# GonzaBerger/bmSparse-SPGEMM-SPMV

Hardware: AMD Instinct MI355X
Metric: bmSparse SpMV fp32 effective GB/s (CSR-convention bytes / time); SpGEMM GFLOP/s under `spgemm` (higher is better)
Workload: dtype f32; 1 GPU; bmSparse SpMV fp32, rmat(scale=20, edge_factor=2)+I, stand-in for webbase-1M; rows=1048576, nnz=3127380, blocks=2073692, x=ones, variant=default (value-stream sweep over the cached plan), hbm_resident_copies_rotated=9

## Files before the change

### bmsparse-spgemm-spmv_amd/csrc/builder.hip

```cpp
#include "matrix.h"
#include "prims.hip.h"
#include <algorithm>
#include <cctype>
#include <memory>
#include <thread>
#include <string>
#include <cstdlib>
#include <cerrno>
#include <cstring>
#include <fcntl.h>
#include <sys/mman.h>
#include <sys/stat.h>
#include <unistd.h>

namespace bmsp {

namespace {
struct MappedFile {
    const char *p = nullptr;
    size_t n = 0;
    int fd = -1;
    ~MappedFile()
    {
        if (p && n) munmap((void *)p, n);
// ... 379 lines not shown
    BMSP_HIP(hipDeviceSynchronize());
    pool_free(m->dense_tiles); m->dense_tiles = nullptr;
    pool_free(m->lane_tiles); m->lane_tiles = nullptr;
    pool_free(m->csr_rowptr); pool_free(m->csr_ent);
    m->csr_rowptr = nullptr; m->csr_ent = nullptr;
    m->values_finite = -1;
    if (!structure_changed) return;
    pool_free(m->rowptr); m->rowptr = nullptr; m->rowptr_rows = 0; m->max_row_blocks = -1;
    m->struct_hash = 0; m->sp_a_hash = 0; m->sp_b_hash = 0;
    m->rm_partner_uid = 0; m->rm_partner_blocks = 0; m->rm_partner_mode = 0; m->rm_partner_cw_hash = 0;
    m->uid = next_matrix_uid();
    pool_free(m->sp_tasks); pool_free(m->sp_task_begin); pool_free(m->sp_c_of_wave);
    m->sp_tasks = nullptr; m->sp_task_begin = nullptr; m->sp_c_of_wave = nullptr; m->sp_n_tasks = 0;
    pool_free(m->spmv_chunks); m->spmv_chunks = nullptr; m->spmv_num_chunks = 0; m->spmv_plan_long = 0; m->spmv_full_tiles = 0;
    pool_free(m->spmv_pos); m->spmv_pos = nullptr; m->spmv_tinfo = nullptr; m->spmv_eoff = nullptr; m->spmv_pos_base = 0; m->spmv_pos_count = 0; m->spmv_pos_tried = 0;
    pool_free(m->spmv_cw); m->spmv_cw = nullptr; m->spmv_cw_chunks = 0; m->spmv_cw_split = 0; m->spmv_cw_tried = 0;
    pool_free(m->block_meta); m->block_meta = nullptr;
    pool_free(m->sym_recs); m->sym_recs = nullptr;
    pool_free(m->col_index); pool_free(m->col_index_row); m->col_index = nullptr; m->col_index_row = nullptr; m->col_index_tried = 0;
    pool_free(m->col_mass); m->col_mass = nullptr;
    pool_free(m->tp_map); m->tp_map = nullptr; m->tp_src_uid = 0; m->tp_permute = 0;
    pool_free(m->add_map); m->add_map = nullptr; m->add_a_uid = 0; m->add_b_uid = 0;
    free_matrix(m->shard_view); m->shard_view = nullptr; m->shard_world = 0; m->shard_rank = 0; m->shard_bounds.clear();
}

void drop_value_caches(bmsp_matrix_s *m)
{
    if (m->dense_tiles || m->lane_tiles || m->csr_rowptr || m->csr_ent) invalidate_matrix(m, 0);
    else m->values_finite = -1;
}

// ... 535 lines not shown
```

### bmsparse-spgemm-spmv_amd/csrc/capi.hip

```cpp
#include "matrix.h"
#include "prims.hip.h"
#include <algorithm>
#include <cmath>
#include <cstdio>
#include <cstdlib>
#include <cstring>
#include <memory>
#include <numeric>
#include <omp.h>
#include <vector>

namespace bmsp {
const std::string &last_error();
void partition_rows(bmsp_matrix_s *A, bmsp_matrix_s *B, int parts, int64_t *bounds, hipStream_t st, uint64_t *total_out = nullptr);
void spgemm_paneled(bmsp_matrix_s *A, bmsp_matrix_s *B, bmsp_matrix_s **C, int mode, int tc_version, int verbose, hipStream_t st,
                    bmsp_spgemm_stats *stats);
bmsp_matrix_s *row_panel(bmsp_matrix_s *m, int64_t rb, int64_t re, hipStream_t st);
bmsp_matrix_s *concat_panels(int num_rows, int num_cols, int parts, const int64_t *block_nums, const int64_t *nnzs,
                             uint64_t *const *d_keys, uint64_t *const *d_bmps, uint64_t *const *d_offsets, void *const *d_values,
                             bmsp_dtype dtype, hipStream_t st);
}

using namespace bmsp;

// ... 540 lines not shown
}

int bmsp_spmv(bmsp_matrix_t A, const void *d_v, void *d_u, int variant, void *stream)
{
    BMSP_API_BEGIN
    need(A, "A");
    spmv(A, d_v, d_u, variant, as_stream(stream));
    BMSP_API_END
}

int bmsp_spmv_launch_info(bmsp_matrix_t A, int variant, char *kernel_name, size_t kernel_name_cap, int64_t *compulsory_bytes, int64_t *format_bytes)
{
    BMSP_API_BEGIN
    need(A, "A");
    spmv_launch_info(A, variant, nullptr, kernel_name, kernel_name_cap, compulsory_bytes, format_bytes);
    BMSP_API_END
}

int bmsp_comm_unique_id(void *id_bytes)
{
    BMSP_API_BEGIN
    need(id_bytes, "id_bytes");
    comm_unique_id(id_bytes);
    BMSP_API_END
}

int bmsp_comm_init(const void *id_bytes, int world, int rank, bmsp_comm_t *out)
{
    BMSP_API_BEGIN
    need(id_bytes, "id_bytes"); need(out, "out");
// ... 394 lines not shown
```

### bmsparse-spgemm-spmv_amd/csrc/matrix.h

```cpp
#ifndef BMSP_MATRIX_H_
#define BMSP_MATRIX_H_

#include "runtime.h"
#include <memory>
#include <vector>

namespace bmsp { uint64_t next_matrix_uid(); }

struct bmsp_matrix_s {
    uint64_t uid = bmsp::next_matrix_uid();
    int num_rows = 0, num_cols = 0;
    int64_t nnz = 0, block_num = 0;
    bmsp_dtype dtype = BMSP_F32;
    int transposed = 0;
    uint64_t *keys = nullptr;
    uint64_t *bmps = nullptr;
    uint64_t *offsets = nullptr;
    void *values = nullptr;
    int ownership = 1;
    uint32_t *rowptr = nullptr;
    int64_t rowptr_rows = 0;
    int64_t max_row_blocks = -1;
    uint32_t *spmv_chunks = nullptr;
    int64_t spmv_num_chunks = 0;
    int64_t spmv_plan_long = 0;
    int64_t spmv_full_tiles = 0;
    size_t spmv_plan_off_cnt = 0, spmv_plan_off_carry = 0;
    uint16_t *spmv_pos = nullptr;
    uint32_t *spmv_tinfo = nullptr;
    uint16_t *spmv_eoff = nullptr;
    int64_t spmv_pos_base = 0, spmv_pos_count = 0;
    int spmv_pos_tried = 0;
    uint32_t *spmv_cw = nullptr;
    int64_t spmv_cw_chunks = 0, spmv_cw_split = 0;
    size_t spmv_cw_off_rec = 0, spmv_cw_off_cnt = 0, spmv_cw_off_carry = 0;
    int spmv_cw_colbits = 0, spmv_cw_tried = 0;
    uint32_t *block_meta = nullptr;
    uint32_t *sym_recs = nullptr;
    uint32_t *col_mass = nullptr;
    uint32_t *col_index = nullptr, *col_index_row = nullptr;
    uint32_t col_index_gran = 0;
    int col_index_tried = 0;
    void *dense_tiles = nullptr;
    uint32_t *csr_rowptr = nullptr, *csr_ent = nullptr;
    void *lane_tiles = nullptr;
    uint64_t rm_partner_uid = 0;
    int64_t rm_partner_blocks = 0;
    int rm_partner_mode = 0;
    int64_t rm_partner_cw_hash = 0;
    uint64_t *sp_tasks = nullptr;
    uint32_t *sp_task_begin = nullptr, *sp_c_of_wave = nullptr;
// ... 117 lines not shown
void prune_check_args(int rule, double tol, int flags, int out_transposed);
void prune_matrix(bmsp_matrix_s *A, int rule, double tol, int flags, int out_transposed, hipStream_t st, bmsp_matrix_s **out,
                  bmsp_prune_stats *stats);
void row_absmax(bmsp_matrix_s *A, void *d_rowmax, hipStream_t st);
void scale_check_args(const void *d_left, const void *d_right, int flags, int out_transposed);
void from_diagonal_check_args(int num_rows, int num_cols, const void *d_diag, bmsp_dtype dtype, int transposed);
void matrix_diagonal(bmsp_matrix_s *A, void *d_diag, hipStream_t st);
bmsp_matrix_s *matrix_from_diagonal(int num_rows, int num_cols, const void *d_diag, bmsp_dtype dtype, int transposed, hipStream_t st);
bmsp_matrix_s *scale_matrix(bmsp_matrix_s *A, const void *d_left, const void *d_right, int flags, int out_transposed, hipStream_t st);
void scale_values_into(bmsp_matrix_s *A, const void *d_left, const void *d_right, int flags, bmsp_matrix_s *out, hipStream_t st);
void prepare_spmv(bmsp_matrix_s *m, hipStream_t st);
void prepare_spgemm_operand(bmsp_matrix_s *m, hipStream_t st);

void spmv(bmsp_matrix_s *A, const void *v, void *u, int variant, hipStream_t st, int64_t row_lo = 0, int64_t row_hi = -1);
void spmv_launch_info(bmsp_matrix_s *A, int variant, hipStream_t st, char *kernel, size_t kernel_cap, int64_t *compulsory, int64_t *format_bytes);
void spmm(bmsp_matrix_s *A, const void *X, int64_t ldx, void *Y, int64_t ldy, int k, hipStream_t st);
void spmm_launch_info(bmsp_matrix_s *A, int k, int64_t ldx, int64_t ldy, hipStream_t st, char *kernel, size_t kernel_cap);
void spgemm(bmsp_matrix_s *A, bmsp_matrix_s *B, bmsp_matrix_s **C, int mode, int tc_version, int verbose, hipStream_t st,
            bmsp_spgemm_stats *stats, bool structure_only = false);
void spgemm_numeric(bmsp_matrix_s *A, bmsp_matrix_s *B, bmsp_matrix_s *C, int tc_version, hipStream_t st, bmsp_spgemm_stats *stats);
template <typename T>
struct PingPong;
bool segsort_tasks_by_column(PingPong<uint64_t> &keys, PingPong<uint64_t> &vals, uint64_t n, int jbits, hipStream_t st, uint64_t max_seg_bound = 0,
                             uint64_t seg_count_bound = 0, int *long_mode = nullptr);
void segsort_check_violation();
void segsort_u64(uint64_t *d_keys, void *d_vals, int val_bytes, int64_t n, const int *d_segs, int64_t num_segs,
                 hipStream_t st);

void comm_unique_id(void *id128);
bmsp_comm_s *comm_init(const void *id128, int world, int rank);
// ... 13 lines not shown
```

### bmsparse-spgemm-spmv_amd/csrc/spmv.hip

```cpp
#include "spmv_plan.h"
#include "prims.hip.h"
#include <cstdlib>
#include <cstdio>
#include <algorithm>
#include <vector>
#include <type_traits>

namespace bmsp {
namespace {

constexpr uint32_t kVsGroup = 96;
bool vstream_eligible(const bmsp_matrix_s *A)
{
    return !(A->spmv_full_tiles * 4 >= A->block_num) && !getenv("BMSP_SPMV_OLD") && A->num_block_cols() < (1ll << 28);
}

struct RowClass {
    const uint32_t *rowptr;
    const uint64_t *offsets;
    uint32_t nbr;
    uint32_t group;
    __device__ bool is_long(uint32_t r) const { return rowptr[r + 1] - rowptr[r] > kItemTiles; }
    __device__ bool starts(uint32_t r) const
    {
// ... 1027 lines not shown
        sum = chunk_fold_batch<1>(carry, ca, ca, cb, r, g);
    } else if (n <= 16u) {
        sum = chunk_fold_batch<2>(carry, ca, ca, cb, r, g);
    } else {
        sum = 0.f;
        for (uint32_t kb = ca; kb <= cb; kb += 32u) sum += chunk_fold_batch<4>(carry, ca, kb, cb, r, g);
    }
    sum += dpp_val<0x111>(0.f, sum);
    sum += dpp_val<0x112>(0.f, sum);
    sum += dpp_val<0x114>(0.f, sum);
    const uint32_t row = br * 8u + r;
    if (g == 7u && row < num_rows) y[row] = sum;
    if (lane == 0) __hip_atomic_store(&counters[ca], 0u, __ATOMIC_RELAXED, __HIP_MEMORY_SCOPE_AGENT);
}

__global__ __launch_bounds__(64, 8) void spmv_chunk_kernel(const ChunkRec *__restrict__ recs, const uint32_t *__restrict__ words,
                                                            const float *__restrict__ values, const float *__restrict__ x, float *__restrict__ y,
                                                            float *__restrict__ carry, uint32_t *__restrict__ counters, uint32_t nnz,
                                                            uint32_t num_rows, uint32_t num_cols, uint32_t colbits)
{
    typedef float f4 __attribute__((ext_vector_type(4)));
    typedef uint32_t u4 __attribute__((ext_vector_type(4)));
    __shared__ __attribute__((aligned(16))) float win[kChWin];
    const int lane = lane_id();
    const uint32_t c = blockIdx.x;
    const ChunkRec rc = recs[c];
    const uint32_t first = c * kChV + (uint32_t)(kChPer * lane);
    const rsrc_t rw = make_rsrc(words, nnz * 4u), rv = make_rsrc(values, nnz * 4u), rx = make_rsrc(x, num_cols * 4u);
    uint32_t w[kChPer];
    float a[kChPer], xv[kChPer];
    if (c * kChV + kChV <= nnz) {
#pragma unroll
        for (int q = 0; q < kChPer; q += 4) {
            const u4 wq = __builtin_bit_cast(u4, __builtin_amdgcn_raw_buffer_load_b128(rw, (first + q) * 4u, 0, 0));
            const f4 aq = __builtin_bit_cast(f4, __builtin_amdgcn_raw_buffer_load_b128(rv, (first + q) * 4u, 0, 0));
#pragma unroll
            for (int i = 0; i < 4; i++) { w[q + i] = wq[i]; a[q + i] = aq[i]; }
        }
    } else {
#pragma unroll
        for (int j = 0; j < kChPer; j++) {
            const uint32_t off = first + j < nnz ? (first + j) * 4u : kOob;
            w[j] = __builtin_amdgcn_raw_buffer_load_b32(rw, off, 0, 0);
            a[j] = Buf<float>::ld(rv, off);
        }
    }
    const uint32_t cmask = (1u << colbits) - 1u;
#pragma unroll
    for (int j = 0; j < kChPer; j++) xv[j] = Buf<float>::ld(rx, first + j < nnz ? (w[j] & cmask) * 4u : kOob);

    float pr[kChPer];
    uint32_t rr[kChPer];
#pragma unroll
    for (int j = 0; j < kChPer; j++) {
        rr[j] = first + j < nnz ? w[j] >> colbits : rc.nwin - 8u;
        pr[j] = first + j < nnz ? a[j] * xv[j] : 0.f;
    }
    if (rc.nwin == 8) {
        float s[8] = {0.f, 0.f, 0.f, 0.f, 0.f, 0.f, 0.f, 0.f};
#pragma unroll
        for (int j = 0; j < kChPer; j++) {
#pragma unroll
            for (int k = 0; k < 8; k++) s[k] += rr[j] == (uint32_t)k ? pr[j] : 0.f;
        }
        const float v = chunk_sum8(s, lane);
        if ((lane & 7) == 0) win[((lane >> 5) & 1) * 4 + ((lane >> 4) & 1) * 2 + ((lane >> 3) & 1)] = v;
    } else {
        for (uint32_t e = (uint32_t)lane; e < rc.nwin; e += 64) win[e] = 0.f;
        __builtin_amdgcn_wave_barrier();
        chunk_seg_reduce(win, rr, pr);
    }
    __builtin_amdgcn_wave_barrier();
    uint32_t ticket = 0;
    if (rc.flags) {
        if ((rc.flags & kChHead) && lane < 8) __hip_atomic_store(&carry[((size_t)c * 2) * 8 + lane], win[lane], __ATOMIC_RELAXED, __HIP_MEMORY_SCOPE_AGENT);
        if ((rc.flags & kChTail) && lane < 8)
            __hip_atomic_store(&carry[((size_t)c * 2 + 1) * 8 + lane], win[rc.nwin - 8u + (uint32_t)lane], __ATOMIC_RELAXED, __HIP_MEMORY_SCOPE_AGENT);
        asm volatile("s_waitcnt vmcnt(0)" ::: "memory");
        if (lane == 0 ? (rc.flags & kChHead) != 0u : lane == 1 && (rc.flags & kChTail) != 0u)
            ticket = __hip_atomic_fetch_add(&counters[lane == 0 ? rc.head_ca : c], 1u, __ATOMIC_RELAXED, __HIP_MEMORY_SCOPE_AGENT);
    }
    const int32_t base = (int32_t)(rc.fb * 8u);
    const uint32_t row_end = min(rc.own_e * 8u, num_rows);
    for (uint32_t row = rc.own_b * 8u + (uint32_t)lane; row < row_end; row += 64) {
        const int32_t rel = (int32_t)row - base;
        y[row] = rel >= 0 && rel < (int32_t)rc.nwin ? win[rel] : 0.f;
    }
    if (!rc.flags) return;
    const uint32_t th = (uint32_t)__builtin_amdgcn_readlane((int)ticket, 0), tt = (uint32_t)__builtin_amdgcn_readlane((int)ticket, 1);
    if ((rc.flags & kChHead) && th == rc.head_cb - rc.head_ca) chunk_fold(carry, y, counters, rc.head_ca, rc.head_cb, rc.fb, num_rows, lane);
    if ((rc.flags & kChTail) && tt == rc.tail_cb - c) chunk_fold(carry, y, counters, c, rc.tail_cb, rc.fb + rc.nwin / 8u - 1u, num_rows, lane);
}

__global__ void chunk_bounds_kernel(const uint64_t *__restrict__ keys, const uint64_t *__restrict__ bmps, const uint64_t *__restrict__ offsets,
                                    uint32_t nb, uint32_t nnz, uint32_t *__restrict__ fbr, uint32_t *__restrict__ lbr)
{
    const uint32_t b = blockIdx.x * blockDim.x + threadIdx.x;
    if (b >= nb) return;
    const uint32_t o = (uint32_t)offsets[b], n = (uint32_t)__popcll(bmps[b]);
    if (n == 0) return;
    const uint32_t br = key_row(keys[b]);
// ... 10 lines not shown
    const uint32_t b = blockIdx.x * blockDim.x + threadIdx.x;
    if (b >= nb) return;
    uint64_t bm = bmps[b];
    const uint64_t k = keys[b];
    const uint32_t br = key_row(k), bc = key_col(k);
    uint32_t idx = (uint32_t)offsets[b];
    while (bm) {
        const uint32_t p = (uint32_t)__clzll((long long)bm);
        bm &= ~(0x8000000000000000ull >> p);
        const uint32_t rel = (br - fbr[idx / kChV]) * 8u + (p >> 3);
        words[idx] = (rel << colbits) | (bc * 8u + (p & 7u));
        idx++;
    }
}

void build_chunk_cache(bmsp_matrix_s *A, hipStream_t st)
{
    if (A->spmv_cw || A->spmv_cw_tried) return;
    A->spmv_cw_tried = 1;
    if (A->dtype != BMSP_F32 || A->view_values_end || A->view_block_begin || A->nnz == 0 || A->nnz >= (1ll << 30) || A->block_num == 0) return;
    if ((uintptr_t)A->values & 15u) return;
    const uint32_t nnz = (uint32_t)A->nnz, nb = (uint32_t)A->block_num;
    const uint32_t nch = (nnz + kChV - 1) / kChV;
    const int colbits = A->num_cols <= 1 ? 1 : 32 - __builtin_clz((uint32_t)A->num_cols - 1u);
    if (colbits > 28) return;
    std::vector<uint32_t> fb(nch), lb(nch);
    {
        DevBuf<uint32_t> d(2 * (size_t)nch);
        hipLaunchKernelGGL(chunk_bounds_kernel, dim3((nb + 255) / 256), dim3(256), 0, st, A->keys, A->bmps, A->offsets, nb, nnz, d.p, d.p + nch);
        BMSP_CHECK_LAUNCH();
        BMSP_HIP(hipStreamSynchronize(st));
        copy_d2h_staged(fb.data(), d.p, 4 * (size_t)nch);
        copy_d2h_staged(lb.data(), d.p + nch, 4 * (size_t)nch);
    }
    const uint64_t row_cap = std::min<uint64_t>(kChWin, 1ull << (32 - colbits));
    std::vector<ChunkRec> rec(nch);
    const uint32_t nbr = (uint32_t)A->num_block_rows();
    int64_t split = 0;
    for (uint32_t c = 0; c < nch; c++) {
        ChunkRec &r = rec[c];
// ... 12 lines not shown
        uint32_t e = c + 1;
        while (e + 1 < nch && fb[e + 1] == lb[c]) e++;
        rec[c].tail_cb = e;
        for (uint32_t k = c + 1; k <= e; k++) { rec[k].head_ca = c; rec[k].head_cb = e; }
    }
    const size_t off_rec = (size_t)nch * kChV * 4, off_cnt = off_rec + sizeof(ChunkRec) * (size_t)nch;
    const size_t off_carry = (off_cnt + 4 * (size_t)nch + 63) & ~size_t(63), total = off_carry + 64 * (size_t)nch;
    char *mem = (char *)pool_alloc(total);
    BMSP_HIP(hipMemsetAsync(mem, 0, total, st));
    BMSP_HIP(hipMemcpyAsync(mem + off_rec, rec.data(), sizeof(ChunkRec) * (size_t)nch, hipMemcpyHostToDevice, st));
    {
        DevBuf<uint32_t> d(nch);
        BMSP_HIP(hipMemcpyAsync(d.p, fb.data(), 4 * (size_t)nch, hipMemcpyHostToDevice, st));
        hipLaunchKernelGGL(chunk_words_kernel, dim3((nb + 255) / 256), dim3(256), 0, st, A->keys, A->bmps, A->offsets, nb, d.p, (uint32_t)colbits, (uint32_t *)mem);
        BMSP_CHECK_LAUNCH();
        BMSP_HIP(hipStreamSynchronize(st));
    }
    A->spmv_cw = (uint32_t *)mem;
    A->spmv_cw_chunks = nch;
    A->spmv_cw_split = split;
    A->spmv_cw_off_rec = off_rec; A->spmv_cw_off_cnt = off_cnt; A->spmv_cw_off_carry = off_carry;
    A->spmv_cw_colbits = colbits;
}

bool chunk_wanted(const bmsp_matrix_s *A, uint32_t row_lo, uint32_t row_hi)
{
    if (A->dtype != BMSP_F32 || row_lo != 0 || row_hi != (uint32_t)A->num_rows || A->view_values_end || A->view_block_begin) return false;
    if (getenv("BMSP_SPMV_NOCHUNK") || getenv("BMSP_SPMV_NO_POSCACHE") || getenv("BMSP_SPMV_RED")) return false;
    if (getenv("BMSP_SPMV_CHUNK")) return true;
    return A->nnz < 2 * A->block_num && (A->nnz + kChV - 1) / kChV >= kChMinChunks;
}

template <typename T>
// ... 24 lines not shown
            const uint32_t passes = pe ? (uint32_t)std::max(1, atoi(pe)) : (groups > 32768 ? 2u : 1u);
            const uint32_t waves = (groups + passes - 1) / passes;
            hipLaunchKernelGGL((spmv_rowgroup_kernel<T, U>), dim3((waves + 3) / 4), dim3(kThreads), 0, st, A->rowptr, A->keys, A->bmps, A->offsets,
                               (const T *)A->values, (const T *)v, (Ac *)u, row_hi, (uint32_t)A->num_cols, nbr,
                               (uint32_t)((size_t)A->values_extent() * sizeof(T)) + 16u, passes, row_lo);
            BMSP_CHECK_LAUNCH();
            return;
        }
        const uint32_t n_items = (uint32_t)A->spmv_num_chunks;
        char *mem = (char *)A->spmv_chunks;
        if constexpr (std::is_same<T, float>::value) {
            if (vstream_eligible(A) && chunk_wanted(A, row_lo, row_hi)) {
                build_chunk_cache(A, st);
                if (A->spmv_cw) {
                    const char *cm = (const char *)A->spmv_cw;
                    hipLaunchKernelGGL(spmv_chunk_kernel, dim3((uint32_t)A->spmv_cw_chunks), dim3(64), 0, st, (const ChunkRec *)(cm + A->spmv_cw_off_rec),
                                       (const uint32_t *)cm, (const float *)A->values, (const float *)v, (float *)u, (float *)(cm + A->spmv_cw_off_carry),
                                       (uint32_t *)(cm + A->spmv_cw_off_cnt), (uint32_t)A->nnz, (uint32_t)A->num_rows, (uint32_t)A->num_cols,
                                       (uint32_t)A->spmv_cw_colbits);
                    BMSP_CHECK_LAUNCH();
                    return;
                }
            }
        }
        if (vstream_eligible(A)) {
            build_pos_cache(A, st);
            const bool cached = A->spmv_pos != nullptr;
            const char *re = getenv("BMSP_SPMV_RED");
            const int red = re ? atoi(re) : (A->nnz < 2 * A->block_num ? kAtomic : kSorted);
#define BMSP_VS_LAUNCH(MODE, RED)                                                                                                                \
    hipLaunchKernelGGL((spmv_vstream_kernel<T, MODE, RED>), dim3(n_items), dim3(64), 0, st, (const SweepItem *)(mem + 64), n_items, A->keys, A->bmps, \
// ... 72 lines not shown
                    if (!vs_single(it)) multi_tiles += (int64_t)(it.blk_end - it.blk_begin);
                    if (it.num_items) long_items++;
                }
                bytes = 32 * n_items + xy + 64 * long_items + es * nv;
                bytes += cached ? 4 * nb + 2 * multi_tiles + 2 * nv : 24 * nb;
            } else {
                name = A->spmv_full_tiles * 4 >= nb ? "spmv_sweep_kernel<FULL>" : "spmv_sweep_kernel";
                bytes = 32 * n_items + 24 * nb + es * nv + xy;
            }
        }
    }
    if (kernel && kernel_cap) snprintf(kernel, kernel_cap, "%s", name);
    if (compulsory) *compulsory = bytes;
}

void prepare_spmv(bmsp_matrix_s *A, hipStream_t st)
{
    if (A->transposed || A->num_block_rows() == 0) return;
    const size_t es = dtype_size(A->dtype);
    if ((size_t)A->values_extent() * es >= (1ull << 32) || (size_t)A->num_cols * es >= (1ull << 32)) return;
    build_plan(A, st);
    const bool rowgroup = A->block_num > 0 && A->nnz >= 16 * A->block_num && A->spmv_plan_long == 0 && !getenv("BMSP_SPMV_NO_ROWGROUP") && pool_owns(A->values);
    if (vstream_eligible(A) && !rowgroup) {
        build_pos_cache(A, st);
        if (chunk_wanted(A, 0, (uint32_t)A->num_rows)) build_chunk_cache(A, st);
    }
}

void spmv(bmsp_matrix_s *A, const void *v, void *u, int variant, hipStream_t st, int64_t row_lo, int64_t row_hi)
{
// ... 17 lines not shown
```

### bmsparse-spgemm-spmv_amd/pybmsp/__init__.py

```python
import ctypes as C
import os
import subprocess
import numpy as np

_PKG = os.path.dirname(os.path.dirname(os.path.abspath(__file__)))
LIB_PATH = os.environ.get("BMSP_LIB_PATH") or os.path.join(_PKG, "lib", "libbmsp.so")

F32, F16, F64 = 0, 1, 2
NP_DTYPE = {F32: np.float32, F16: np.float16, F64: np.float64}
OUT_DTYPE = {F32: np.float32, F16: np.float32, F64: np.float64}
SORT_AUTO, SORT_SEGMENTED, SORT_GLOBAL = 0, 1, 2
SPMV_DEFAULT, SPMV_BATCHED = 0, 1
PRUNE_ABS, PRUNE_ROW_REL = 0, 1
PRUNE_KEEP_DIAGONAL = 1
SCALE_DIV_LEFT, SCALE_DIV_RIGHT = 1, 2
_PRUNE_RULES = {"abs": PRUNE_ABS, "row_rel": PRUNE_ROW_REL, PRUNE_ABS: PRUNE_ABS, PRUNE_ROW_REL: PRUNE_ROW_REL}

SYMBOLS = [
    "bmsp_last_error", "bmsp_version", "bmsp_device_count", "bmsp_set_device", "bmsp_malloc", "bmsp_free",
    "bmsp_memcpy_h2d", "bmsp_memcpy_d2h", "bmsp_memcpy_d2d", "bmsp_memset", "bmsp_synchronize", "bmsp_trim_pool",
    "bmsp_event_create", "bmsp_event_record", "bmsp_event_elapsed_ms", "bmsp_event_destroy",
    "bmsp_matrix_from_mtx", "bmsp_matrix_from_coo", "bmsp_matrix_from_coo_device", "bmsp_matrix_from_arrays",
    "bmsp_matrix_save", "bmsp_matrix_load", "bmsp_matrix_free", "bmsp_matrix_prepare", "bmsp_matrix_invalidate", "bmsp_matrix_info", "bmsp_matrix_arrays", "bmsp_matrix_block_row_ptr",
    "bmsp_matrix_transpose", "bmsp_matrix_convert_layout", "bmsp_matrix_copy_values", "bmsp_matrix_add", "bmsp_matrix_add_values",
    "bmsp_matrix_prune", "bmsp_matrix_row_absmax",
    "bmsp_matrix_diagonal", "bmsp_matrix_from_diagonal", "bmsp_matrix_scale", "bmsp_matrix_scale_values",
    "bmsp_matrix_to_coo_host", "bmsp_matrix_to_coo_device", "bmsp_matrix_to_csr_device", "bmsp_matrix_from_csr_device", "bmsp_matrix_compare", "bmsp_matrix_compare_device", "bmsp_spmv", "bmsp_spmv_launch_info", "bmsp_spmm", "bmsp_spmm_launch_info", "bmsp_spgemm", "bmsp_spgemm_symbolic", "bmsp_spgemm_numeric", "bmsp_selftest_mfma_layout", "bmsp_selftest_mfma_f32_chain", "bmsp_selftest_tile_product", "bmsp_selftest_mfma_f32_cancel", "bmsp_segsort_u64",
    "bmsp_partition_rows", "bmsp_matrix_row_panel", "bmsp_matrix_concat_panels",
    "bmsp_comm_unique_id", "bmsp_comm_init", "bmsp_comm_init_from_env", "bmsp_comm_init_loopback", "bmsp_shard_layout", "bmsp_shard_row_slices", "bmsp_comm_info", "bmsp_comm_free", "bmsp_spgemm_sharded", "bmsp_spgemm_sharded_ex", "bmsp_spmv_sharded",
    "bmsp_csr_from_mtx", "bmsp_csr_from_arrays", "bmsp_csr_info", "bmsp_csr_arrays", "bmsp_csr_multiply",
    "bmsp_csr_spmv", "bmsp_csr_multiply_host", "bmsp_csr_spmv_host", "bmsp_csr_free",
]


class BmspError(RuntimeError):
    def __init__(self, status, msg):
        super().__init__("bmsp status %d: %s" % (status, msg))
        self.status = status


class SpgemmStats(C.Structure):
    _fields_ = [("task_list_size", C.c_int64), ("bmp_reduction", C.c_int64), ("surviving_tasks", C.c_int64),
# ... 69 lines not shown
        L.bmsp_matrix_prune.argtypes = [vp, i, C.c_double, i, i, vp, p(vp), p(PruneStats)]
        L.bmsp_matrix_row_absmax.argtypes = [vp, vp, vp]
        L.bmsp_matrix_diagonal.argtypes = [vp, vp, vp]
        L.bmsp_matrix_from_diagonal.argtypes = [i, i, vp, i, i, vp, p(vp)]
        L.bmsp_matrix_scale.argtypes = [vp, vp, vp, i, i, vp, p(vp)]
        L.bmsp_matrix_scale_values.argtypes = [vp, vp, vp, i, vp, vp]
        L.bmsp_matrix_to_coo_host.argtypes = [vp, vp, vp, vp]
        L.bmsp_matrix_to_coo_device.argtypes = [vp, vp, vp, vp, vp]
        L.bmsp_matrix_to_csr_device.argtypes = [vp, vp, vp, vp, vp]
        L.bmsp_matrix_from_csr_device.argtypes = [i, i, i64, vp, vp, vp, i, i, vp, p(vp)]
        L.bmsp_matrix_compare_device.argtypes = [vp, i64, vp, vp, vp, p(C.c_double), p(i64), vp]
        L.bmsp_matrix_compare.argtypes = [vp, i64, vp, vp, vp, p(C.c_double), p(i64)]
        L.bmsp_spmv.argtypes = [vp, vp, vp, i, vp]
        L.bmsp_spmm.argtypes = [vp, vp, i64, vp, i64, i, vp]
        L.bmsp_spmv_launch_info.argtypes = [vp, i, C.c_char_p, C.c_size_t, p(i64), p(i64)]
        L.bmsp_spmm_launch_info.argtypes = [vp, i, i64, i64, C.c_char_p, C.c_size_t]
        L.bmsp_spgemm.argtypes = [vp, vp, p(vp), i, i, i, vp, p(SpgemmStats)]
        L.bmsp_spgemm_symbolic.argtypes = [vp, vp, p(vp), i, i, vp, p(SpgemmStats)]
        L.bmsp_spgemm_numeric.argtypes = [vp, vp, vp, i, vp, p(SpgemmStats)]
        L.bmsp_selftest_mfma_layout.argtypes = [p(i)]
        L.bmsp_selftest_mfma_f32_chain.argtypes = [p(i)]
        L.bmsp_selftest_tile_product.argtypes = [p(i)]
        L.bmsp_selftest_mfma_f32_cancel.argtypes = [p(i), p(i)]
        L.bmsp_segsort_u64.argtypes = [vp, vp, i, i64, vp, i64, vp]
        L.bmsp_partition_rows.argtypes = [vp, vp, i, vp]
        L.bmsp_matrix_row_panel.argtypes = [vp, i64, i64, p(vp)]
        L.bmsp_matrix_concat_panels.argtypes = [i, i, i, vp, vp, vp, vp, vp, vp, i, p(vp)]
        L.bmsp_comm_unique_id.argtypes = [vp]
        L.bmsp_comm_init.argtypes = [vp, i, i, p(vp)]
        L.bmsp_comm_init_from_env.argtypes = [p(vp)]
# ... 378 lines not shown
def spmv(A, v, u=None, batched=False, stream=None):
    i = A.info()
    if u is None:
        u = DeviceArray(i["num_rows"], OUT_DTYPE[i["dtype"]])
    check(lib().bmsp_spmv(A.h, v.ptr, u.ptr, SPMV_BATCHED if batched else SPMV_DEFAULT, stream))
    return u


def spmv_launch_info(A, variant=0):
    name = C.create_string_buffer(128)
    cb, fb = C.c_int64(), C.c_int64()
    check(lib().bmsp_spmv_launch_info(A.h, int(variant), name, 128, C.byref(cb), C.byref(fb)))
    return {"kernel": name.value.decode(), "compulsory_bytes": cb.value, "format_bytes": fb.value}


def spmm(A, X, k, Y=None, ldx=None, ldy=None, stream=None):
    i = A.info()
    ldx = k if ldx is None else ldx
    ldy = k if ldy is None else ldy
    if Y is None:
        Y = DeviceArray(i["num_rows"] * ldy, OUT_DTYPE[i["dtype"]])
    check(lib().bmsp_spmm(A.h, X.ptr, int(ldx), Y.ptr, int(ldy), int(k), stream))
    return Y


def spmm_launch_info(A, k, ldx=None, ldy=None):
    name = C.create_string_buffer(160)
    check(lib().bmsp_spmm_launch_info(A.h, int(k), int(k if ldx is None else ldx), int(k if ldy is None else ldy), name, 160))
    return name.value.decode()

# ... 183 lines not shown
```

### include/bmsp.h

```cpp
#ifndef BMSP_H_
#define BMSP_H_

#include <stddef.h>
#include <stdint.h>

#ifdef __cplusplus
extern "C" {
#endif

#define BMSP_BLOCK_WIDTH 8
#define BMSP_BLOCK_HEIGHT 8

typedef enum {
    BMSP_OK = 0,
    BMSP_ERR_INVALID = -1,
    BMSP_ERR_IO = -2,
    BMSP_ERR_HIP = -3,
    BMSP_ERR_NOMEM = -4,
    BMSP_ERR_UNSUPPORTED = -5,
    BMSP_ERR_LIMIT = -6
} bmsp_status;

typedef enum { BMSP_F32 = 0, BMSP_F16 = 1, BMSP_F64 = 2 } bmsp_dtype;

// ... 77 lines not shown
                                const double *d_vals, int transposed, bmsp_dtype dtype, void *stream, bmsp_matrix_t *out);

int bmsp_matrix_compare(bmsp_matrix_t m, int64_t nnz, const int *rows, const int *cols, const double *vals,
                        double *mean_rel_err, int64_t *missing);
int bmsp_matrix_compare_device(bmsp_matrix_t m, int64_t nnz, const int *d_rows, const int *d_cols, const double *d_vals,
                               double *mean_rel_err, int64_t *missing, void *stream);


#define BMSP_SPMV_DEFAULT 0
#define BMSP_SPMV_BATCHED 1

int bmsp_spmv(bmsp_matrix_t A, const void *d_v, void *d_u, int variant, void *stream);

int bmsp_spmv_launch_info(bmsp_matrix_t A, int variant, char *kernel_name, size_t kernel_name_cap, int64_t *compulsory_bytes, int64_t *format_bytes);

int bmsp_spmm(bmsp_matrix_t A, const void *d_X, int64_t ldx, void *d_Y, int64_t ldy, int k, void *stream);

int bmsp_spmm_launch_info(bmsp_matrix_t A, int k, int64_t ldx, int64_t ldy, char *kernel_name, size_t kernel_name_cap);

typedef struct {
    int64_t task_list_size;
    int64_t bmp_reduction;
    int64_t surviving_tasks;
    int64_t c_blocks;
    int64_t c_nnz;
    double t_us[10];
    int sort_path;
    int mac_kernel;
    int mac_variant;
    int sort_long;
// ... 86 lines not shown
```

Measured before the change: 2930 GB/s.

## Row-sort chunk words at plan build and reduce with a segmented scan

Adds a build-time kernel that sorts each 512-entry chunk's packed words by row and stores the original position, segment-start bit and a row-presence bitmap in the spare high bits. A templated sorted variant of the chunk SpMV kernel uses these to replace the per-chunk window zeroing and scattered segmented reduction with a wave-wide run-sum, and resolves row sums through a popcount-compacted LDS table. Values still stream in their original order and are permuted through LDS. It is enabled by default when the column count fits in 20 bits, with an env switch to disable it, and it adds more LDS indexing and bit manipulation per element.

```diff
diff --git a/bmsparse-spgemm-spmv_amd/csrc/builder.hip b/bmsparse-spgemm-spmv_amd/csrc/builder.hip
--- a/bmsparse-spgemm-spmv_amd/csrc/builder.hip
+++ b/bmsparse-spgemm-spmv_amd/csrc/builder.hip
@@ -417,7 +417,7 @@
     m->sp_tasks = nullptr; m->sp_task_begin = nullptr; m->sp_c_of_wave = nullptr; m->sp_n_tasks = 0;
     pool_free(m->spmv_chunks); m->spmv_chunks = nullptr; m->spmv_num_chunks = 0; m->spmv_plan_long = 0; m->spmv_full_tiles = 0;
     pool_free(m->spmv_pos); m->spmv_pos = nullptr; m->spmv_tinfo = nullptr; m->spmv_eoff = nullptr; m->spmv_pos_base = 0; m->spmv_pos_count = 0; m->spmv_pos_tried = 0;
-    pool_free(m->spmv_cw); m->spmv_cw = nullptr; m->spmv_cw_chunks = 0; m->spmv_cw_split = 0; m->spmv_cw_tried = 0;
+    pool_free(m->spmv_cw); m->spmv_cw = nullptr; m->spmv_cw_chunks = 0; m->spmv_cw_split = 0; m->spmv_cw_tried = 0; m->spmv_cw_layout = 0;
     pool_free(m->block_meta); m->block_meta = nullptr;
     pool_free(m->sym_recs); m->sym_recs = nullptr;
     pool_free(m->col_index); pool_free(m->col_index_row); m->col_index = nullptr; m->col_index_row = nullptr; m->col_index_tried = 0;
diff --git a/bmsparse-spgemm-spmv_amd/csrc/capi.hip b/bmsparse-spgemm-spmv_amd/csrc/capi.hip
--- a/bmsparse-spgemm-spmv_amd/csrc/capi.hip
+++ b/bmsparse-spgemm-spmv_amd/csrc/capi.hip
@@ -578,6 +578,14 @@
     BMSP_API_BEGIN
     need(A, "A");
     spmv_launch_info(A, variant, nullptr, kernel_name, kernel_name_cap, compulsory_bytes, format_bytes);
+    BMSP_API_END
+}
+
+int bmsp_spmv_chunk_layout(bmsp_matrix_t A, int *layout)
+{
+    BMSP_API_BEGIN
+    need(A, "A"); need(layout, "layout");
+    *layout = spmv_chunk_layout(A, nullptr);
     BMSP_API_END
 }
 
diff --git a/bmsparse-spgemm-spmv_amd/csrc/matrix.h b/bmsparse-spgemm-spmv_amd/csrc/matrix.h
--- a/bmsparse-spgemm-spmv_amd/csrc/matrix.h
+++ b/bmsparse-spgemm-spmv_amd/csrc/matrix.h
@@ -34,7 +34,7 @@
     uint32_t *spmv_cw = nullptr;
     int64_t spmv_cw_chunks = 0, spmv_cw_split = 0;
     size_t spmv_cw_off_rec = 0, spmv_cw_off_cnt = 0, spmv_cw_off_carry = 0;
-    int spmv_cw_colbits = 0, spmv_cw_tried = 0;
+    int spmv_cw_colbits = 0, spmv_cw_tried = 0, spmv_cw_layout = 0;
     uint32_t *block_meta = nullptr;
     uint32_t *sym_recs = nullptr;
     uint32_t *col_mass = nullptr;
@@ -182,6 +182,7 @@
 
 void spmv(bmsp_matrix_s *A, const void *v, void *u, int variant, hipStream_t st, int64_t row_lo = 0, int64_t row_hi = -1);
 void spmv_launch_info(bmsp_matrix_s *A, int variant, hipStream_t st, char *kernel, size_t kernel_cap, int64_t *compulsory, int64_t *format_bytes);
+int spmv_chunk_layout(bmsp_matrix_s *A, hipStream_t st);
 void spmm(bmsp_matrix_s *A, const void *X, int64_t ldx, void *Y, int64_t ldy, int k, hipStream_t st);
 void spmm_launch_info(bmsp_matrix_s *A, int k, int64_t ldx, int64_t ldy, hipStream_t st, char *kernel, size_t kernel_cap);
 void spgemm(bmsp_matrix_s *A, bmsp_matrix_s *B, bmsp_matrix_s **C, int mode, int tc_version, int verbose, hipStream_t st,
diff --git a/bmsparse-spgemm-spmv_amd/csrc/spmv.hip b/bmsparse-spgemm-spmv_amd/csrc/spmv.hip
--- a/bmsparse-spgemm-spmv_amd/csrc/spmv.hip
+++ b/bmsparse-spgemm-spmv_amd/csrc/spmv.hip
@@ -1,6 +1,7 @@
 #include "spmv_plan.h"
 #include "prims.hip.h"
 #include <cstdlib>
+#include <cstring>
 #include <cstdio>
 #include <algorithm>
 #include <vector>
@@ -1065,6 +1066,96 @@
     if (lane == 0) __hip_atomic_store(&counters[ca], 0u, __ATOMIC_RELAXED, __HIP_MEMORY_SCOPE_AGENT);
 }
 
+constexpr int kChSortedColbits = 20;
+constexpr uint32_t kChT = kChV + 64;
+constexpr uint32_t kChSortedLds = kChT + 64;
+static_assert(kChSortedLds * 4 <= 6144, "the row-sorted form keeps to 6 KB of LDS per wave");
+
+__device__ __forceinline__ float chunk_row_value(const float *T, const uint32_t *bmw, const uint32_t *pre, uint32_t e)
+{
+    const uint32_t wd = bmw[e >> 5], sh = e & 31u;
+    const float v = T[pre[e >> 5] + (uint32_t)__popc(wd & ((1u << sh) - 1u))];
+    return (wd >> sh) & 1u ? v : 0.f;
+}
+
+template <bool WHOLE>
+__device__ __forceinline__ void chunk_sorted_reduce(float *lds, const uint32_t *__restrict__ words, const float *__restrict__ values,
+                                                    const float *__restrict__ x, uint32_t c, uint32_t nnz, uint32_t num_cols, uint32_t colbits, int lane)
+{
+    typedef float f4 __attribute__((ext_vector_type(4)));
+    typedef uint32_t u4 __attribute__((ext_vector_type(4)));
+    const uint32_t first = c * kChV + (uint32_t)(kChPer * lane), nval = WHOLE ? kChV : nnz - c * kChV;
+    const rsrc_t rw = make_rsrc(words, (uint32_t)min((uint64_t)gridDim.x * kChV * 4u, (uint64_t)0xfffffffcu));
+    const rsrc_t rv = make_rsrc(values, nnz * 4u), rx = make_rsrc(x, num_cols * 4u);
+    uint32_t w[kChPer];
+    float a[kChPer], xv[kChPer];
+#pragma unroll
+    for (int q = 0; q < kChPer; q += 4) {
+        const u4 wq = __builtin_bit_cast(u4, __builtin_amdgcn_raw_buffer_load_b128(rw, (first + q) * 4u, 0, 0));
+#pragma unroll
+        for (int i = 0; i < 4; i++) w[q + i] = wq[i];
+    }
+    if constexpr (WHOLE) {
+#pragma unroll
+        for (int q = 0; q < kChPer; q += 4) {
+            const f4 aq = __builtin_bit_cast(f4, __builtin_amdgcn_raw_buffer_load_b128(rv, (first + q) * 4u, 0, 0));
+#pragma unroll
+            for (int i = 0; i < 4; i++) a[q + i] = aq[i];
+        }
+    } else {
+#pragma unroll
+        for (int j = 0; j < kChPer; j++) a[j] = Buf<float>::ld(rv, first + j < nnz ? (first + j) * 4u : kOob);
+    }
+    const uint32_t cmask = (1u << colbits) - 1u;
+#pragma unroll
+    for (int j = 0; j < kChPer; j++) xv[j] = Buf<float>::ld(rx, WHOLE || (uint32_t)(kChPer * lane + j) < nval ? (w[j] & cmask) * 4u : kOob);
+    float *T = lds;
+    uint32_t *bmw = (uint32_t *)(lds + kChT), *pre = bmw + 32;
+    chunk_put8(T + kChPer * lane, a);
+    uint32_t bits = 0;
+#pragma unroll
+    for (int j = 0; j < kChPer; j++) bits |= (w[j] >> (colbits + 10u)) << (2 * j);
+    ((uint16_t *)bmw)[lane] = (uint16_t)bits;
+    __builtin_amdgcn_wave_barrier();
+    float pr[kChPer];
+#pragma unroll
+    for (int j = 0; j < kChPer; j++) pr[j] = T[(w[j] >> colbits) & (kChV - 1u)];
+    {
+        const uint32_t wd = lane < 32 ? bmw[lane] : 0u, pc = (uint32_t)__popc(wd);
+        const uint32_t below = wave_inclusive_sum_dpp(pc) - pc;
+        if (lane < 32) pre[lane] = below;
+    }
+    uint32_t st[kChPer], k[kChPer], tot = 0;
+#pragma unroll
+    for (int j = 0; j < kChPer; j++) {
+        st[j] = (w[j] >> (colbits + 9u)) & 1u;
+        tot += st[j];
+        k[j] = tot;
+    }
+    const uint32_t base = wave_inclusive_sum_dpp(tot) - tot - 1u;
+#pragma unroll
+    for (int j = 0; j < kChPer; j++) {
+        k[j] += base;
+        pr[j] = WHOLE || (uint32_t)(kChPer * lane + j) < nval ? pr[j] * xv[j] : 0.f;
+    }
+    float t = pr[0];
+#pragma unroll
+    for (int j = 1; j < kChPer; j++) t = st[j] ? pr[j] : t + pr[j];
+    const float run = wave_run_sum(t, k[kChPer - 1]);
+    const float left = dpp_val<0x138>(0.f, run);
+    const uint32_t st_right = dpp_u32<0x130>(1u, st[0]);
+    __builtin_amdgcn_wave_barrier();
+    const uint32_t dump = kChV + (uint32_t)lane;
+    float acc = st[0] ? pr[0] : left + pr[0];
+#pragma unroll
+    for (int j = 1; j < kChPer; j++) {
+        T[st[j] ? (k[j - 1] & (kChV - 1u)) : dump] = acc;
+        acc = st[j] ? pr[j] : acc + pr[j];
+    }
+    T[st_right ? (k[kChPer - 1] & (kChV - 1u)) : dump] = acc;
+}
+
+template <bool SORTED>
 __global__ __launch_bounds__(64, 8) void spmv_chunk_kernel(const ChunkRec *__restrict__ recs, const uint32_t *__restrict__ words,
                                                             const float *__restrict__ values, const float *__restrict__ x, float *__restrict__ y,
                                                             float *__restrict__ carry, uint32_t *__restrict__ counters, uint32_t nnz,
@@ -1072,61 +1163,70 @@
 {
     typedef float f4 __attribute__((ext_vector_type(4)));
     typedef uint32_t u4 __attribute__((ext_vector_type(4)));
-    __shared__ __attribute__((aligned(16))) float win[kChWin];
+    __shared__ __attribute__((aligned(16))) float win[SORTED ? kChSortedLds : kChWin];
     const int lane = lane_id();
     const uint32_t c = blockIdx.x;
     const ChunkRec rc = recs[c];
-    const uint32_t first = c * kChV + (uint32_t)(kChPer * lane);
-    const rsrc_t rw = make_rsrc(words, nnz * 4u), rv = make_rsrc(values, nnz * 4u), rx = make_rsrc(x, num_cols * 4u);
-    uint32_t w[kChPer];
-    float a[kChPer], xv[kChPer];
-    if (c * kChV + kChV <= nnz) {
-#pragma unroll
-        for (int q = 0; q < kChPer; q += 4) {
-            const u4 wq = __builtin_bit_cast(u4, __builtin_amdgcn_raw_buffer_load_b128(rw, (first + q) * 4u, 0, 0));
-            const f4 aq = __builtin_bit_cast(f4, __builtin_amdgcn_raw_buffer_load_b128(rv, (first + q) * 4u, 0, 0));
-#pragma unroll
-            for (int i = 0; i < 4; i++) { w[q + i] = wq[i]; a[q + i] = aq[i]; }
-        }
+    if constexpr (SORTED) {
+        if (c * kChV + kChV <= nnz) chunk_sorted_reduce<true>(win, words, values, x, c, nnz, num_cols, colbits, lane);
+        else chunk_sorted_reduce<false>(win, words, values, x, c, nnz, num_cols, colbits, lane);
     } else {
+        const uint32_t first = c * kChV + (uint32_t)(kChPer * lane);
+        const rsrc_t rw = make_rsrc(words, nnz * 4u), rv = make_rsrc(values, nnz * 4u), rx = make_rsrc(x, num_cols * 4u);
+        uint32_t w[kChPer];
+        float a[kChPer], xv[kChPer];
+        if (c * kChV + kChV <= nnz) {
+#pragma unroll
+            for (int q = 0; q < kChPer; q += 4) {
+                const u4 wq = __builtin_bit_cast(u4, __builtin_amdgcn_raw_buffer_load_b128(rw, (first + q) * 4u, 0, 0));
+                const f4 aq = __builtin_bit_cast(f4, __builtin_amdgcn_raw_buffer_load_b128(rv, (first + q) * 4u, 0, 0));
+#pragma unroll
+                for (int i = 0; i < 4; i++) { w[q + i] = wq[i]; a[q + i] = aq[i]; }
+            }
+        } else {
+#pragma unroll
+            for (int j = 0; j < kChPer; j++) {
+                const uint32_t off = first + j < nnz ? (first + j) * 4u : kOob;
+                w[j] = __builtin_amdgcn_raw_buffer_load_b32(rw, off, 0, 0);
+                a[j] = Buf<float>::ld(rv, off);
+            }
+        }
+        const uint32_t cmask = (1u << colbits) - 1u;
+#pragma unroll
+        for (int j = 0; j < kChPer; j++) xv[j] = Buf<float>::ld(rx, first + j < nnz ? (w[j] & cmask) * 4u : kOob);
+
+        float pr[kChPer];
+        uint32_t rr[kChPer];
 #pragma unroll
         for (int j = 0; j < kChPer; j++) {
-            const uint32_t off = first + j < nnz ? (first + j) * 4u : kOob;
-            w[j] = __builtin_amdgcn_raw_buffer_load_b32(rw, off, 0, 0);
-            a[j] = Buf<float>::ld(rv, off);
-        }
-    }
-    const uint32_t cmask = (1u << colbits) - 1u;
-#pragma unroll
-    for (int j = 0; j < kChPer; j++) xv[j] = Buf<float>::ld(rx, first + j < nnz ? (w[j] & cmask) * 4u : kOob);
-
-    float pr[kChPer];
-    uint32_t rr[kChPer];
-#pragma unroll
-    for (int j = 0; j < kChPer; j++) {
-        rr[j] = first + j < nnz ? w[j] >> colbits : rc.nwin - 8u;
-        pr[j] = first + j < nnz ? a[j] * xv[j] : 0.f;
-    }
-    if (rc.nwin == 8) {
-        float s[8] = {0.f, 0.f, 0.f, 0.f, 0.f, 0.f, 0.f, 0.f};
-#pragma unroll
-        for (int j = 0; j < kChPer; j++) {
-#pragma unroll
-            for (int k = 0; k < 8; k++) s[k] += rr[j] == (uint32_t)k ? pr[j] : 0.f;
-        }
-        const float v = chunk_sum8(s, lane);
-        if ((lane & 7) == 0) win[((lane >> 5) & 1) * 4 + ((lane >> 4) & 1) * 2 + ((lane >> 3) & 1)] = v;
-    } else {
-        for (uint32_t e = (uint32_t)lane; e < rc.nwin; e += 64) win[e] = 0.f;
-        __builtin_amdgcn_wave_barrier();
-        chunk_seg_reduce(win, rr, pr);
+            rr[j] = first + j < nnz ? w[j] >> colbits : rc.nwin - 8u;
+            pr[j] = first + j < nnz ? a[j] * xv[j] : 0.f;
+        }
+        if (rc.nwin == 8) {
+            float s[8] = {0.f, 0.f, 0.f, 0.f, 0.f, 0.f, 0.f, 0.f};
+#pragma unroll
+            for (int j = 0; j < kChPer; j++) {
+#pragma unroll
+                for (int k = 0; k < 8; k++) s[k] += rr[j] == (uint32_t)k ? pr[j] : 0.f;
+            }
+            const float v = chunk_sum8(s, lane);
+            if ((lane & 7) == 0) win[((lane >> 5) & 1) * 4 + ((lane >> 4) & 1) * 2 + ((lane >> 3) & 1)] = v;
+        } else {
+            for (uint32_t e = (uint32_t)lane; e < rc.nwin; e += 64) win[e] = 0.f;
+            __builtin_amdgcn_wave_barrier();
+            chunk_seg_reduce(win, rr, pr);
+        }
     }
     __builtin_amdgcn_wave_barrier();
+    const auto row_sum = [&](uint32_t rel) -> float {
+        if constexpr (SORTED) return chunk_row_value(win, (const uint32_t *)(win + kChT), (const uint32_t *)(win + kChT) + 32, rel);
+        else return win[rel];
+    };
     uint32_t ticket = 0;
     if (rc.flags) {
-        if ((rc.flags & kChHead) && lane < 8) __hip_atomic_store(&carry[((size_t)c * 2) * 8 + lane], win[lane], __ATOMIC_RELAXED, __HIP_MEMORY_SCOPE_AGENT);
+        if ((rc.flags & kChHead) && lane < 8) __hip_atomic_store(&carry[((size_t)c * 2) * 8 + lane], row_sum((uint32_t)lane), __ATOMIC_RELAXED, __HIP_MEMORY_SCOPE_AGENT);
         if ((rc.flags & kChTail) && lane < 8)
-            __hip_atomic_store(&carry[((size_t)c * 2 + 1) * 8 + lane], win[rc.nwin - 8u + (uint32_t)lane], __ATOMIC_RELAXED, __HIP_MEMORY_SCOPE_AGENT);
+            __hip_atomic_store(&carry[((size_t)c * 2 + 1) * 8 + lane], row_sum(rc.nwin - 8u + (uint32_t)lane), __ATOMIC_RELAXED, __HIP_MEMORY_SCOPE_AGENT);
         asm volatile("s_waitcnt vmcnt(0)" ::: "memory");
         if (lane == 0 ? (rc.flags & kChHead) != 0u : lane == 1 && (rc.flags & kChTail) != 0u)
             ticket = __hip_atomic_fetch_add(&counters[lane == 0 ? rc.head_ca : c], 1u, __ATOMIC_RELAXED, __HIP_MEMORY_SCOPE_AGENT);
@@ -1135,7 +1235,13 @@
     const uint32_t row_end = min(rc.own_e * 8u, num_rows);
     for (uint32_t row = rc.own_b * 8u + (uint32_t)lane; row < row_end; row += 64) {
         const int32_t rel = (int32_t)row - base;
-        y[row] = rel >= 0 && rel < (int32_t)rc.nwin ? win[rel] : 0.f;
+        const bool in = rel >= 0 && rel < (int32_t)rc.nwin;
+        if constexpr (SORTED) {
+            const float v = row_sum(in ? (uint32_t)rel : 0u);
+            y[row] = in ? v : 0.f;
+        } else {
+            y[row] = in ? win[rel] : 0.f;
+        }
     }
     if (!rc.flags) return;
     const uint32_t th = (uint32_t)__builtin_amdgcn_readlane((int)ticket, 0), tt = (uint32_t)__builtin_amdgcn_readlane((int)ticket, 1);
@@ -1176,6 +1282,34 @@
     }
 }
 
+__global__ __launch_bounds__(kChV) void chunk_sort_kernel(uint32_t *__restrict__ words, uint32_t nnz, uint32_t colbits)
+{
+    typedef uint32_t u4 __attribute__((ext_vector_type(4)));
+    __shared__ __attribute__((aligned(16))) uint32_t keys[kChV];
+    __shared__ uint32_t out[kChV], srow[kChV], bm[kChWin / 32];
+    const uint32_t c = blockIdx.x, i = threadIdx.x, n = min(nnz - c * kChV, kChV);
+    const uint32_t w = words[(size_t)c * kChV + i];
+    const uint32_t r = w >> colbits, key = i < n ? (r << 9) | i : ~0u;
+    keys[i] = key;
+    out[i] = 0;
+    srow[i] = ~0u;
+    if (i < kChWin / 32) bm[i] = 0;
+    __syncthreads();
+    if (i < n) {
+        uint32_t pos = 0;
+        for (uint32_t j = 0; j < kChV / 4; j++) {
+            const u4 q = ((const u4 *)keys)[j];
+            pos += (q[0] < key ? 1u : 0u) + (q[1] < key ? 1u : 0u) + (q[2] < key ? 1u : 0u) + (q[3] < key ? 1u : 0u);
+        }
+        out[pos] = (w & ((1u << colbits) - 1u)) | (i << colbits);
+        srow[pos] = r;
+        atomicOr(&bm[(r >> 5) & (kChWin / 32 - 1)], 1u << (r & 31u));
+    }
+    __syncthreads();
+    const uint32_t start = i < n && (i == 0 || srow[i] != srow[i - 1]) ? 1u : 0u;
+    words[(size_t)c * kChV + i] = out[i] | (start << (colbits + 9u)) | (((bm[i >> 4] >> ((2u * i) & 31u)) & 3u) << (colbits + 10u));
+}
+
 void build_chunk_cache(bmsp_matrix_s *A, hipStream_t st)
 {
     if (A->spmv_cw || A->spmv_cw_tried) return;
@@ -1186,6 +1320,8 @@
     const uint32_t nch = (nnz + kChV - 1) / kChV;
     const int colbits = A->num_cols <= 1 ? 1 : 32 - __builtin_clz((uint32_t)A->num_cols - 1u);
     if (colbits > 28) return;
+    const char *se = getenv("BMSP_SPMV_CHUNK_SORTED");
+    const bool sorted = kChV == 512 && kChWin == 1024 && colbits <= kChSortedColbits && !(se && atoi(se) == 0);
     std::vector<uint32_t> fb(nch), lb(nch);
     {
         DevBuf<uint32_t> d(2 * (size_t)nch);
@@ -1228,9 +1364,14 @@
         BMSP_HIP(hipMemcpyAsync(d.p, fb.data(), 4 * (size_t)nch, hipMemcpyHostToDevice, st));
         hipLaunchKernelGGL(chunk_words_kernel, dim3((nb + 255) / 256), dim3(256), 0, st, A->keys, A->bmps, A->offsets, nb, d.p, (uint32_t)colbits, (uint32_t *)mem);
         BMSP_CHECK_LAUNCH();
+        if (sorted) {
+            hipLaunchKernelGGL(chunk_sort_kernel, dim3(nch), dim3(kChV), 0, st, (uint32_t *)mem, nnz, (uint32_t)colbits);
+            BMSP_CHECK_LAUNCH();
+        }
         BMSP_HIP(hipStreamSynchronize(st));
     }
     A->spmv_cw = (uint32_t *)mem;
+    A->spmv_cw_layout = sorted ? 2 : 1;
     A->spmv_cw_chunks = nch;
     A->spmv_cw_split = split;
     A->spmv_cw_off_rec = off_rec; A->spmv_cw_off_cnt = off_cnt; A->spmv_cw_off_carry = off_carry;
@@ -1285,7 +1426,7 @@
                 build_chunk_cache(A, st);
                 if (A->spmv_cw) {
                     const char *cm = (const char *)A->spmv_cw;
-                    hipLaunchKernelGGL(spmv_chunk_kernel, dim3((uint32_t)A->spmv_cw_chunks), dim3(64), 0, st, (const ChunkRec *)(cm + A->spmv_cw_off_rec),
+                    hipLaunchKernelGGL(A->spmv_cw_layout == 2 ? spmv_chunk_kernel<true> : spmv_chunk_kernel<false>, dim3((uint32_t)A->spmv_cw_chunks), dim3(64), 0, st, (const ChunkRec *)(cm + A->spmv_cw_off_rec),
                                        (const uint32_t *)cm, (const float *)A->values, (const float *)v, (float *)u, (float *)(cm + A->spmv_cw_off_carry),
                                        (uint32_t *)(cm + A->spmv_cw_off_cnt), (uint32_t)A->nnz, (uint32_t)A->num_rows, (uint32_t)A->num_cols,
                                        (uint32_t)A->spmv_cw_colbits);
@@ -1388,6 +1529,13 @@
     if (compulsory) *compulsory = bytes;
 }
 
+int spmv_chunk_layout(bmsp_matrix_s *A, hipStream_t st)
+{
+    char name[64];
+    spmv_launch_info(A, BMSP_SPMV_DEFAULT, st, name, sizeof(name), nullptr, nullptr);
+    return strcmp(name, "spmv_chunk_kernel") == 0 ? A->spmv_cw_layout : 0;
+}
+
 void prepare_spmv(bmsp_matrix_s *A, hipStream_t st)
 {
     if (A->transposed || A->num_block_rows() == 0) return;
diff --git a/bmsparse-spgemm-spmv_amd/pybmsp/__init__.py b/bmsparse-spgemm-spmv_amd/pybmsp/__init__.py
--- a/bmsparse-spgemm-spmv_amd/pybmsp/__init__.py
+++ b/bmsparse-spgemm-spmv_amd/pybmsp/__init__.py
@@ -25,7 +25,7 @@
     "bmsp_matrix_transpose", "bmsp_matrix_convert_layout", "bmsp_matrix_copy_values", "bmsp_matrix_add", "bmsp_matrix_add_values",
     "bmsp_matrix_prune", "bmsp_matrix_row_absmax",
     "bmsp_matrix_diagonal", "bmsp_matrix_from_diagonal", "bmsp_matrix_scale", "bmsp_matrix_scale_values",
-    "bmsp_matrix_to_coo_host", "bmsp_matrix_to_coo_device", "bmsp_matrix_to_csr_device", "bmsp_matrix_from_csr_device", "bmsp_matrix_compare", "bmsp_matrix_compare_device", "bmsp_spmv", "bmsp_spmv_launch_info", "bmsp_spmm", "bmsp_spmm_launch_info", "bmsp_spgemm", "bmsp_spgemm_symbolic", "bmsp_spgemm_numeric", "bmsp_selftest_mfma_layout", "bmsp_selftest_mfma_f32_chain", "bmsp_selftest_tile_product", "bmsp_selftest_mfma_f32_cancel", "bmsp_segsort_u64",
+    "bmsp_matrix_to_coo_host", "bmsp_matrix_to_coo_device", "bmsp_matrix_to_csr_device", "bmsp_matrix_from_csr_device", "bmsp_matrix_compare", "bmsp_matrix_compare_device", "bmsp_spmv", "bmsp_spmv_launch_info", "bmsp_spmv_chunk_layout", "bmsp_spmm", "bmsp_spmm_launch_info", "bmsp_spgemm", "bmsp_spgemm_symbolic", "bmsp_spgemm_numeric", "bmsp_selftest_mfma_layout", "bmsp_selftest_mfma_f32_chain", "bmsp_selftest_tile_product", "bmsp_selftest_mfma_f32_cancel", "bmsp_segsort_u64",
     "bmsp_partition_rows", "bmsp_matrix_row_panel", "bmsp_matrix_concat_panels",
     "bmsp_comm_unique_id", "bmsp_comm_init", "bmsp_comm_init_from_env", "bmsp_comm_init_loopback", "bmsp_shard_layout", "bmsp_shard_row_slices", "bmsp_comm_info", "bmsp_comm_free", "bmsp_spgemm_sharded", "bmsp_spgemm_sharded_ex", "bmsp_spmv_sharded",
     "bmsp_csr_from_mtx", "bmsp_csr_from_arrays", "bmsp_csr_info", "bmsp_csr_arrays", "bmsp_csr_multiply",
@@ -125,6 +125,7 @@
         L.bmsp_spmv.argtypes = [vp, vp, vp, i, vp]
         L.bmsp_spmm.argtypes = [vp, vp, i64, vp, i64, i, vp]
         L.bmsp_spmv_launch_info.argtypes = [vp, i, C.c_char_p, C.c_size_t, p(i64), p(i64)]
+        L.bmsp_spmv_chunk_layout.argtypes = [vp, p(i)]
         L.bmsp_spmm_launch_info.argtypes = [vp, i, i64, i64, C.c_char_p, C.c_size_t]
         L.bmsp_spgemm.argtypes = [vp, vp, p(vp), i, i, i, vp, p(SpgemmStats)]
         L.bmsp_spgemm_symbolic.argtypes = [vp, vp, p(vp), i, i, vp, p(SpgemmStats)]
@@ -533,6 +534,12 @@
     return {"kernel": name.value.decode(), "compulsory_bytes": cb.value, "format_bytes": fb.value}
 
 
+def spmv_chunk_layout(A):
+    out = C.c_int()
+    check(lib().bmsp_spmv_chunk_layout(A.h, C.byref(out)))
+    return out.value
+
+
 def spmm(A, X, k, Y=None, ldx=None, ldy=None, stream=None):
     i = A.info()
     ldx = k if ldx is None else ldx
diff --git a/include/bmsp.h b/include/bmsp.h
--- a/include/bmsp.h
+++ b/include/bmsp.h
@@ -115,6 +115,8 @@
 
 int bmsp_spmv_launch_info(bmsp_matrix_t A, int variant, char *kernel_name, size_t kernel_name_cap, int64_t *compulsory_bytes, int64_t *format_bytes);
 
+int bmsp_spmv_chunk_layout(bmsp_matrix_t A, int *layout);
+
 int bmsp_spmm(bmsp_matrix_t A, const void *d_X, int64_t ldx, void *d_Y, int64_t ldy, int k, void *stream);
 
 int bmsp_spmm_launch_info(bmsp_matrix_t A, int k, int64_t ldx, int64_t ldy, char *kernel_name, size_t kernel_name_cap);
```

Measured after the change: 2982 GB/s (median of 6 runs). 1.8% higher.
